# EricLBuehler/diffusion-rs

Measured on AMD Instinct MI355X. Metric: images/sec, FLUX.1-dev 1024x1024 50-step, higher is better.
Workload: dtype bf16; 1 GPU; FLUX.1-dev bf16 1024x1024 50-step, batch=1 per GPU, S=4096 img + T=512 txt tokens, step = one image (50x Flux::forward + Euler, unpack, VAE decode, u8); global_batch=1, parallelism=single GPU

## Files before the change

diffusion-rs_amd/_lib.py:

```python
import ctypes as C
import os

_HERE = os.path.dirname(os.path.abspath(__file__))
LIB_PATH = os.environ.get("FMI_LIB") or os.path.join(_HERE, "libflux_mi355x.so")
ALT_LIB_PATH = os.path.join(_HERE, "libflux_mi355x_alt.so")


class FmiError(RuntimeError):

    def __init__(self, msg, code=None):
        super().__init__(msg)
        self.code = code


ERR_INVALID, ERR_HIP, ERR_STATE, ERR_UNSUPPORTED, ERR_NOMEM = -1, -2, -3, -4, -5


class FluxConfig(C.Structure):
    _fields_ = [("in_channels", C.c_int), ("pooled_projection_dim", C.c_int), ("joint_attention_dim", C.c_int),
                ("num_attention_heads", C.c_int), ("num_layers", C.c_int), ("num_single_layers", C.c_int),
                ("guidance_embeds", C.c_int), ("axes_dim", C.c_int * 3), ("theta", C.c_int)]


ALL_TO_ALL_FN = C.CFUNCTYPE(C.c_int, C.c_void_p, C.c_void_p, C.c_void_p, C.c_size_t, C.c_void_p)
# ... 239 lines not shown
    lib.fmi_linear_int8_bf16.argtypes = [C.c_void_p, C.c_void_p, C.c_void_p, C.c_void_p, C.c_void_p, C.c_int, C.c_int, C.c_int, C.c_int, C.c_void_p]
    lib.fmi_sdpa_bf16.argtypes = [C.c_void_p, C.c_void_p, C.c_void_p, C.c_void_p, C.c_int, C.c_int, C.c_int, C.c_int, C.c_int, C.c_float, C.c_int,
                                  C.c_void_p]
    lib.fmi_sdpa_fp8qk.argtypes = lib.fmi_sdpa_bf16.argtypes
    lib.fmi_sdpa_workspace_bytes.argtypes = [C.c_int, C.c_int, C.c_int]
    lib.fmi_sdpa_workspace_bytes.restype = C.c_size_t
    lib.fmi_sdpa_bf16_ws.argtypes = [C.c_void_p] * 4 + [C.c_int] * 5 + [C.c_float, C.c_int, C.c_void_p, C.c_size_t, C.c_void_p]
    lib.fmi_sdpa_fp8qk_ws.argtypes = [C.c_void_p] * 4 + [C.c_int] * 5 + [C.c_float, C.c_int, C.c_int, C.c_void_p, C.c_size_t, C.c_void_p]
    lib.fmi_sdpa_fp8.argtypes = [C.c_void_p] * 4 + [C.c_int] * 5 + [C.c_float, C.c_int, C.c_float, C.c_int, C.c_void_p]
    lib.fmi_sdpa_fp8_ws.argtypes = [C.c_void_p] * 4 + [C.c_int] * 5 + [C.c_float, C.c_int, C.c_float, C.c_int, C.c_void_p, C.c_size_t, C.c_void_p]
    lib.fmi_linear_q8_workspace_bytes.argtypes = [C.c_int, C.c_int]
    lib.fmi_linear_q8_workspace_bytes.restype = C.c_size_t
    lib.fmi_linear_fp8_ws.argtypes = list(lib.fmi_linear_fp8.argtypes[:-1]) + [C.c_void_p, C.c_size_t, C.c_void_p]
    lib.fmi_linear_i8_ws.argtypes = lib.fmi_linear_fp8_ws.argtypes
    lib.fmi_layernorm_mod.argtypes = [C.c_void_p, C.c_void_p, C.c_void_p, C.c_void_p, C.c_int, C.c_int, C.c_float, C.c_void_p]
    lib.fmi_groupnorm_nhwc.argtypes = [C.c_void_p, C.c_void_p, C.c_void_p, C.c_void_p, C.c_int, C.c_int, C.c_int, C.c_int, C.c_float, C.c_int,
                                       C.c_void_p]
    lib.fmi_conv2d_nhwc.argtypes = [C.c_void_p, C.c_void_p, C.c_void_p, C.c_void_p, C.c_void_p, C.c_int, C.c_int, C.c_int, C.c_int, C.c_int,
                                    C.c_int, C.c_int, C.c_void_p]
    for name in ("f32", "f16", "bf16"):
        for q in ("int8", "fp4", "nf4"):
            getattr(lib, f"dequantize_blockwise_{name}_{q}").argtypes = [C.c_void_p, C.c_void_p, C.c_void_p, C.c_void_p, C.c_int, C.c_int, C.c_void_p]
            getattr(lib, f"dequantize_blockwise_{name}_{q}").restype = None
        getattr(lib, f"dequantize_8bit_kernel_{name}").argtypes = [C.c_void_p, C.c_void_p, C.c_void_p, C.c_int, C.c_int, C.c_int]
        getattr(lib, f"dequantize_8bit_kernel_{name}").restype = None
    lib.fmi_event_create.argtypes = [C.POINTER(C.c_void_p)]
    lib.fmi_event_record.argtypes = [C.c_void_p, C.c_void_p]
    lib.fmi_event_elapsed_ms.argtypes = [C.c_void_p, C.c_void_p, C.POINTER(C.c_float)]
    lib.fmi_event_destroy.argtypes = [C.c_void_p]
    lib.fmi_stream_synchronize.argtypes = [C.c_void_p]
# ... 22 lines not shown


EXPORTED = [
    "fmi_last_error", "fmi_abi_version", "fmi_init", "fmi_device_info", "fmi_build_id", "fmi_has_alt_kernels", "fmi_flux_default_config", "fmi_flux_create", "fmi_flux_destroy",
    "fmi_flux_set_tensor", "fmi_flux_set_linear_bnb4", "fmi_flux_set_linear_int8", "fmi_flux_set_linear_gguf", "fmi_gguf_block_info", "fmi_gguf_dequantize", "fmi_flux_get_tensor", "fmi_flux_lora_add", "fmi_flux_lora_set_weight", "fmi_flux_lora_remove", "fmi_flux_lora_count", "fmi_flux_lora_name", "fmi_flux_set_quant_dense_cache", "fmi_flux_set_sequence_parallel", "fmi_flux_set_split_k", "fmi_set_bnb4_onewave_min_rows", "fmi_flux_set_attention_rescale_threshold", "fmi_flux_set_attention_kernel", "fmi_flux_state_buffer_count", "fmi_flux_state_export", "fmi_flux_state_adopt", "fmi_flux_state_buffer", "fmi_flux_set_modulation_gemm", "fmi_flux_quantize_fp8", "fmi_flux_quantize_int8", "fmi_flux_calibrate_int8", "fmi_flux_set_fp8_attention", "fmi_flux_missing_count", "fmi_flux_missing_name", "fmi_flux_size_in_bytes",
    "fmi_flux_forward", "fmi_flux_denoise", "fmi_flux_denoise_inpaint", "fmi_flux_forward_context", "fmi_flux_denoise_context", "fmi_flux_denoise_cached", "fmi_flux_step_cache_bytes", "fmi_flux_denoise_cfg", "fmi_flux_create_cond", "fmi_flux_cond_channels", "fmi_flux_forward_control", "fmi_flux_denoise_control", "fmi_flux_denoise_with",
    "fmi_flux_create_controlnet", "fmi_flux_is_controlnet", "fmi_flux_forward_controlnet", "fmi_flux_denoise_controlnet", "fmi_flux_controlnet_eval", "fmi_flux_controlnet_sample", "fmi_add_scaled_rows_bf16",
    "fmi_flux_set_profiling", "fmi_flux_set_fused_qkv_relayout", "fmi_flux_phase_count", "fmi_flux_phase_name", "fmi_flux_phase_ms",
    "fmi_vae_default_config", "fmi_vae_create", "fmi_vae_destroy", "fmi_vae_set_tensor", "fmi_vae_missing_count", "fmi_vae_missing_name",
    "fmi_vae_scale_factor", "fmi_vae_shift_factor", "fmi_vae_decode", "fmi_vae_encode", "fmi_vae_mid_attention",
    "fmi_t5_default_config", "fmi_t5_create", "fmi_t5_destroy", "fmi_t5_set_tensor", "fmi_t5_set_linear_bnb4", "fmi_t5_set_linear_int8", "fmi_t5_missing_count", "fmi_t5_missing_name",
    "fmi_t5_size_in_bytes", "fmi_t5_forward", "fmi_clip_default_config", "fmi_clip_create", "fmi_clip_destroy", "fmi_clip_set_tensor",
    "fmi_clip_missing_count", "fmi_clip_missing_name", "fmi_clip_size_in_bytes", "fmi_clip_forward", "fmi_pack_latents", "fmi_unpack_latents", "fmi_postprocess_u8",
    "fmi_preprocess_u8", "fmi_latent_mask", "fmi_encode_latents", "fmi_scale_noise", "fmi_latent_ids", "fmi_cfg_euler_step", "fmi_cast_cols_bf16", "fmi_mask_image", "fmi_fill_condition",
    "fmi_randn", "fmi_philox_u32", "fmi_calculate_shift", "fmi_get_timesteps", "fmi_linear_bf16", "fmi_linear_bnb4_bf16", "fmi_linear_int8_bf16", "fmi_quantize_rows_fp8", "fmi_linear_fp8", "fmi_quantize_rows_i8", "fmi_linear_i8", "fmi_gemm_q8", "fmi_quantize_rows_i8_asym", "fmi_rowsum_i8", "fmi_quantize_rows_i8_scaled", "fmi_col_absmax", "fmi_gemm_i8_asym", "fmi_gemm_group", "fmi_splitk_resid_gate", "fmi_set_gemm_kernel", "fmi_linear_q8_workspace_bytes", "fmi_linear_fp8_ws", "fmi_linear_i8_ws", "fmi_sdpa_bf16", "fmi_sdpa_fp8qk", "fmi_sdpa_workspace_bytes", "fmi_sdpa_bf16_ws", "fmi_sdpa_fp8qk_ws", "fmi_sdpa_fp8", "fmi_sdpa_fp8_ws", "fmi_set_attention_kernel", "fmi_layernorm_mod",
    "fmi_release_scratch", "fmi_timestep_embedding", "fmi_rope_table", "fmi_rmsnorm_rope",
    "fmi_groupnorm_nhwc", "fmi_conv2d_nhwc",
    "fmi_comm_probe", "fmi_comm_unique_id", "fmi_comm_create", "fmi_comm_destroy", "fmi_comm_rank", "fmi_comm_world_size", "fmi_comm_stats", "fmi_comm_all_to_all",
    "fmi_comm_broadcast", "fmi_comm_gather",
    "dequantize_blockwise_f32_int8", "dequantize_blockwise_f32_fp4", "dequantize_blockwise_f32_nf4", "dequantize_blockwise_f16_int8",
    "dequantize_blockwise_f16_fp4", "dequantize_blockwise_f16_nf4", "dequantize_blockwise_bf16_int8", "dequantize_blockwise_bf16_fp4",
    "dequantize_blockwise_bf16_nf4", "dequantize_8bit_kernel_f32", "dequantize_8bit_kernel_f16", "dequantize_8bit_kernel_bf16",
    "fmi_malloc", "fmi_free", "fmi_memcpy", "fmi_memset", "fmi_stream_synchronize", "fmi_event_create", "fmi_event_record",
    "fmi_event_elapsed_ms", "fmi_event_destroy",
]
```

diffusion-rs_amd/csrc/capi.hip:

```cpp
#include <algorithm>
#include <cmath>
#include <cstring>
#include <map>
#include <mutex>
#include <set>
#include <thread>
#include <tuple>
#include <utility>
#include <vector>

#include "common.h"

namespace fmi {
static thread_local std::string g_err;
void set_error(const std::string& msg) { g_err = msg; }
int fail(fmi_status st, const std::string& msg) {
  g_err = msg;
  return (int)st;
}
}
using namespace fmi;

extern "C" const char* fmi_last_error(void) { return g_err.c_str(); }
extern "C" int fmi_abi_version(void) { return FMI_ABI_VERSION; }
// ... 467 lines not shown
  return fmi_sdpa_fp8_ws(q, k, v, o, B, H, Lq, Lk, d, scale, score_exp2, v_scale, out_token_major, ws.p, bytes, stream);
}

extern "C" int fmi_set_attention_kernel(int kind) {
  if (kind < 0 || kind > 5) return fail(FMI_ERR_INVALID, "set_attention_kernel: kind must be 0 .. 5");
  if (!alt_kernels_built() && kind != 5 && kind != 1)
    return fail(FMI_ERR_UNSUPPORTED, "set_attention_kernel: this build carries kernels 5 and 1; 0, 2, 3, 4 live in the test build (libflux_mi355x_alt.so: make alt)");
  set_attention_kind(kind);
  return FMI_OK;
}

extern "C" int fmi_layernorm_mod(const float* x, const float* scale, const float* shift, void* out_bf16, int rows, int D, float eps, void* stream) {
  if (!x || !out_bf16) return fail(FMI_ERR_INVALID, "layernorm_mod: null pointer");
  return launch_layernorm_mod(x, scale, shift, 0, 0, (bf16_t*)out_bf16, rows, D, eps, (hipStream_t)stream);
}

extern "C" int fmi_timestep_embedding(const float* t, int B, int dim, float* out, void* stream) {
  if (!t || !out) return fail(FMI_ERR_INVALID, "timestep_embedding: null pointer");
  if (B <= 0 || dim <= 0 || dim % 2) return fail(FMI_ERR_INVALID, "timestep_embedding: B > 0 and an even dim > 0 required");
  return launch_timestep_embedding(t, B, dim, out, (hipStream_t)stream);
}
extern "C" int fmi_rope_table(const float* txt_ids, const float* img_ids, int B, int T, int S, const int* axes_dim, int theta, float* pe, void* stream) {
  if (!axes_dim || !pe || (T > 0 && !txt_ids) || (S > 0 && !img_ids)) return fail(FMI_ERR_INVALID, "rope_table: null pointer");
  if (B <= 0 || T < 0 || S < 0 || T + S == 0) return fail(FMI_ERR_INVALID, "rope_table: empty problem");
  for (int a = 0; a < 3; ++a)
    if (axes_dim[a] <= 0 || axes_dim[a] % 2) return fail(FMI_ERR_INVALID, "rope_table: every axes_dim must be positive and even");
  if (theta <= 0) return fail(FMI_ERR_INVALID, "rope_table: theta must be positive");
  return launch_rope_table(txt_ids, img_ids, B, T, S, axes_dim, theta, pe, (hipStream_t)stream);
}
extern "C" int fmi_rmsnorm_rope(const void* q, const void* k, int ld, const void* q_weight, const void* k_weight, const float* pe, void* q_out, void* k_out,
// ... 18 lines not shown
```

diffusion-rs_amd/csrc/common.h:

```cpp
#pragma once
#ifndef FMI_ALT_KERNELS
#define FMI_ALT_KERNELS 0
#endif
#include <type_traits>
#include <hip/hip_runtime.h>
#include <stdint.h>

#include <set>
#include <string>
#include <vector>

#include "../../include/flux_mi355x.h"

namespace fmi {

void set_error(const std::string& msg);
int fail(fmi_status st, const std::string& msg);
#define FMI_HIP_TRY(expr)                                                                       \
  do {                                                                                          \
    hipError_t _e = (expr);                                                                     \
    if (_e != hipSuccess)                                                                       \
      return ::fmi::fail(FMI_ERR_HIP, std::string(#expr) + ": " + hipGetErrorString(_e) + " @" + \
                                          __FILE__ + ":" + std::to_string(__LINE__));           \
  } while (0)
// ... 306 lines not shown
                        const bf16_t* wk, const float* pe, int64_t pe_bstride, bf16_t* qo, bf16_t* ko,
                        int B, int H, int rows, int row_off, int Ltot, hipStream_t stream);
int launch_qk_norm_rope_f32(const bf16_t* q, const bf16_t* k, int ld, int64_t in_bstride, const bf16_t* wq, const bf16_t* wk, const float* pe,
                            int64_t pe_bstride, float* qo, float* ko, int B, int H, int rows, int row_off, int Ltot, hipStream_t stream);
int launch_rope_table(const float* txt_ids, const float* img_ids, int B, int T, int S, const int* axes,
                      int theta, float* pe, hipStream_t stream, const float* ctx_ids = nullptr, int R = 0);
int launch_layernorm_mod2(const float* x, const float* scale, const float* shift, int mod_bstride, int rows_per_batch, bf16_t* out, int rows,
                          const float* x2, const float* scale2, const float* shift2, int rows_per_batch2, bf16_t* out2, int rows2, int D, float eps,
                          hipStream_t stream);
int launch_layernorm_mod_fp8_2(const float* x, const float* scale, const float* shift, int mod_bstride, int rows_per_batch, uint8_t* out,
                               float* out_scale, int rows, const float* x2, const float* scale2, const float* shift2, int rows_per_batch2, uint8_t* out2,
                               float* out_scale2, int rows2, int D, float eps, hipStream_t stream, int kind = 1, const float* smooth = nullptr,
                               const float* smooth2 = nullptr);
int launch_layernorm_mod(const float* x, const float* scale, const float* shift, int mod_bstride,
                         int rows_per_batch, bf16_t* out, int rows, int D, float eps, hipStream_t stream);
int launch_quantize_rows_fp8(const bf16_t* x, int ld, int rows, int K, uint8_t* out, float* scale, hipStream_t stream, int kind = 1, const float* vec = nullptr);
int launch_quantize_rows_i8_asym(const bf16_t* x, int ld, int rows, int K, int d0, uint8_t* out, float* scale, float* offset, hipStream_t stream, const float* vec = nullptr);
int launch_rowsum_i8(const int8_t* wq, const float* w_scale, int N, int K, int d0, float* w_sum, hipStream_t stream);
int launch_layernorm_mod_fp8(const float* x, const float* scale, const float* shift, int mod_bstride, int rows_per_batch,
                             uint8_t* out, float* out_scale, int rows, int D, float eps, hipStream_t stream, int kind = 1, const float* smooth = nullptr);
int launch_col_absmax(const bf16_t* x, int ld, int rows, int K, float* amax, hipStream_t stream);
void smooth_factors_host(const float* act_amax, const float* w_amax, int K, float* s_out, float* inv_out);
int launch_gemv(const float* x, const bf16_t* W, const bf16_t* bias, float* y, int M, int N, int K,
                int silu_in, int accumulate, hipStream_t stream);
int launch_dequant_int8_scb_bf16(const int8_t* w, const float* scb, bf16_t* out, int col, int64_t n, hipStream_t stream);
constexpr int LORA_TILE_ROWS = 64, LORA_RANK_CHUNK = 16;
int launch_lora_pack(const float* A, const float* B, int rows, int K, int r, double coef, float* Acat, double* Bt, int rows_pad, int off, hipStream_t stream);
int launch_lora_merge(const bf16_t* w0, bf16_t* w, int rows, int K, const float* A, const double* Bt, int rows_pad, int Rpad, hipStream_t stream);
int launch_timestep_embedding(const float* t, int B, int dim, float* out, hipStream_t stream);
int launch_cast_to_bf16(const void* src, fmi_dtype dt, bf16_t* dst, int64_t n, hipStream_t stream);
// ... 22 lines not shown
```

diffusion-rs_amd/csrc/fp8.hip:

```cpp
#include <algorithm>
#include <cmath>
#include <vector>

#include "common.h"

namespace fmi {

namespace {

constexpr float kE4M3Max = 448.0f;
constexpr float kI8Max = 127.0f;

__device__ __forceinline__ float block_max_256(float v, float* red) {
  v = wave_max(v);
  if ((threadIdx.x & 63) == 0) red[threadIdx.x >> 6] = v;
  __syncthreads();
  return fmaxf(fmaxf(red[0], red[1]), fmaxf(red[2], red[3]));
}

__device__ __forceinline__ uint32_t pack_e4m3x4(float a, float b, float c, float d) {
  int v = 0;
  v = __builtin_amdgcn_cvt_pk_fp8_f32(a, b, v, false);
  v = __builtin_amdgcn_cvt_pk_fp8_f32(c, d, v, true);
  return (uint32_t)v;
// ... 128 lines not shown
  const int4* r = reinterpret_cast<const int4*>(wq + (int64_t)n * K);
  int t = 0;
  for (int i = (d0 >> 4) + lane; i < (K >> 4); i += 64) {
    const int4 x = r[i];
    const int w[4] = {x.x, x.y, x.z, x.w};
#pragma unroll
    for (int e = 0; e < 4; ++e) t += (int)(int8_t)(w[e] & 0xff) + (int)(int8_t)((w[e] >> 8) & 0xff) + (int)(int8_t)((w[e] >> 16) & 0xff) + (w[e] >> 24);
  }
#pragma unroll
  for (int o = 32; o > 0; o >>= 1) t += __shfl_xor(t, o);
  if (lane == 0) w_sum[n] = w_scale[n] * (float)t;
}

constexpr int LN_MAXV = 4;

template <bool I8>
__global__ __launch_bounds__(256) void layernorm_mod_fp8_kernel(const float* __restrict x1, const float* __restrict scale1,
                                                                const float* __restrict shift1, int mod_bstride, int rows_per_batch1,
                                                                uint8_t* __restrict out1, float* __restrict out_scale1, int D, float eps, int rows1,
                                                                const float* __restrict x2, const float* __restrict scale2,
                                                                const float* __restrict shift2, int rows_per_batch2, uint8_t* __restrict out2,
                                                                float* __restrict out_scale2, const float* __restrict smooth1,
                                                                const float* __restrict smooth2) {
  __shared__ float red[2][4];
  __shared__ float redm[4];
  const bool second = (int)blockIdx.x >= rows1;
  const int row = second ? blockIdx.x - rows1 : blockIdx.x;
  const float* x = second ? x2 : x1;
  const float* scale = second ? scale2 : scale1;
  const float* shift = second ? shift2 : shift1;
// ... 53 lines not shown
      v[c] = make_float4(a, b, cc, d);
      am = fmaxf(fmaxf(am, fmaxf(fabsf(a), fabsf(b))), fmaxf(fabsf(cc), fabsf(d)));
    }
  }
  am = fmaxf(block_max_256(am, redm), 1e-30f);
  constexpr float QMAX = I8 ? kI8Max : kE4M3Max;
  const float inv = QMAX / am;
  if (threadIdx.x == 0) out_scale[row] = am / QMAX;
  uint32_t* o = reinterpret_cast<uint32_t*>(out + (int64_t)row * D);
#pragma unroll
  for (int c = 0; c < LN_MAXV; ++c) {
    const int i = threadIdx.x + c * 256;
    if (i < nv) o[i] = pack_q8x4<I8>(v[c].x * inv, v[c].y * inv, v[c].z * inv, v[c].w * inv);
  }
}


__global__ __launch_bounds__(256) void col_absmax_kernel(const bf16_t* __restrict x, int ld, int rows, int chunks, float* __restrict amax) {
  const int i = blockIdx.x * 256 + threadIdx.x;
  if (i >= chunks) return;
  float m[8] = {0.f, 0.f, 0.f, 0.f, 0.f, 0.f, 0.f, 0.f};
  for (int r = blockIdx.y; r < rows; r += gridDim.y) {
    const uint4 raw = *reinterpret_cast<const uint4*>(x + (int64_t)r * ld + 8 * i);
    float f[8];
    widen8<false>(raw, nullptr, 0, f);
#pragma unroll
    for (int e = 0; e < 8; ++e) m[e] = fmaxf(m[e], fabsf(f[e]));
  }
#pragma unroll
  for (int e = 0; e < 8; ++e)
// ... 26 lines not shown
}
int launch_rowsum_i8(const int8_t* wq, const float* w_scale, int N, int K, int d0, float* w_sum, hipStream_t stream) {
  if (N <= 0) return FMI_OK;
  if (K % 16 || d0 % 16 || d0 < 0 || d0 > K) return fail(FMI_ERR_INVALID, "rowsum_i8: K and d0 must be multiples of 16");
  hipLaunchKernelGGL(rowsum_i8_kernel, dim3((N + 3) / 4), dim3(256), 0, stream, wq, w_scale, N, K, d0, w_sum);
  FMI_LAUNCH_CHECK();
  return FMI_OK;
}

int launch_layernorm_mod_fp8_2(const float* x, const float* scale, const float* shift, int mod_bstride, int rows_per_batch, uint8_t* out,
                               float* out_scale, int rows, const float* x2, const float* scale2, const float* shift2, int rows_per_batch2, uint8_t* out2,
                               float* out_scale2, int rows2, int D, float eps, hipStream_t stream, int kind, const float* smooth, const float* smooth2) {
  if (rows + rows2 <= 0) return FMI_OK;
  if (kind != 1 && kind != 2) return fail(FMI_ERR_INVALID, "layernorm_mod_fp8: kind must be 1 (e4m3) or 2 (int8)");
  if (D % 4 || D > 256 * 4 * LN_MAXV) return fail(FMI_ERR_INVALID, "layernorm_mod_fp8: D must be a multiple of 4 and <= 4096");
  if (kind == 2)
    hipLaunchKernelGGL(layernorm_mod_fp8_kernel<true>, dim3(rows + rows2), dim3(256), 0, stream, x, scale, shift, mod_bstride, rows_per_batch, out, out_scale,
                       D, eps, rows, x2, scale2, shift2, rows_per_batch2, out2, out_scale2, smooth, smooth2);
  else
    hipLaunchKernelGGL(layernorm_mod_fp8_kernel<false>, dim3(rows + rows2), dim3(256), 0, stream, x, scale, shift, mod_bstride, rows_per_batch, out, out_scale,
                       D, eps, rows, x2, scale2, shift2, rows_per_batch2, out2, out_scale2, smooth, smooth2);
  FMI_LAUNCH_CHECK();
  return FMI_OK;
}
int launch_layernorm_mod_fp8(const float* x, const float* scale, const float* shift, int mod_bstride, int rows_per_batch, uint8_t* out,
                             float* out_scale, int rows, int D, float eps, hipStream_t stream, int kind, const float* smooth) {
  return launch_layernorm_mod_fp8_2(x, scale, shift, mod_bstride, rows_per_batch, out, out_scale, rows, nullptr, nullptr, nullptr, 0, nullptr, nullptr, 0,
                                    D, eps, stream, kind, smooth, nullptr);
}

int launch_col_absmax(const bf16_t* x, int ld, int rows, int K, float* amax, hipStream_t stream) {
  if (rows <= 0 || K <= 0) return FMI_OK;
  if (K % 8 || ld % 8) return fail(FMI_ERR_INVALID, "col_absmax: K and ld must be multiples of 8");
  const int chunks = K / 8, rblocks = std::min((rows + 63) / 64, 512);
  hipLaunchKernelGGL(col_absmax_kernel, dim3((chunks + 255) / 256, rblocks), dim3(256), 0, stream, x, ld, rows, chunks, amax);
  FMI_LAUNCH_CHECK();
// ... 21 lines not shown
```

diffusion-rs_amd/csrc/norm_rope.hip:

```cpp
#include "common.h"

namespace fmi {

template <bool REG>
__global__ __launch_bounds__(256) void layernorm_mod_kernel(const float* __restrict x1, const float* __restrict scale1,
                                                            const float* __restrict shift1, int mod_bstride, int rows_per_batch1,
                                                            bf16_t* __restrict out1, int D, float eps, int rows1, const float* __restrict x2,
                                                            const float* __restrict scale2, const float* __restrict shift2, int rows_per_batch2,
                                                            bf16_t* __restrict out2) {
  __shared__ float red[2][4];
  const bool second = (int)blockIdx.x >= rows1;
  const int row = second ? blockIdx.x - rows1 : blockIdx.x;
  const float* x = second ? x2 : x1;
  const float* scale = second ? scale2 : scale1;
  const float* shift = second ? shift2 : shift1;
  const int rows_per_batch = second ? rows_per_batch2 : rows_per_batch1;
  bf16_t* out = second ? out2 : out1;
  const float4* xr = reinterpret_cast<const float4*>(x + (int64_t)row * D);
  const int nv = D >> 2;
  constexpr int MAXV = 4;
  float4 keep[MAXV], ksc[MAXV], ksh[MAXV];
  float s = 0.f, s2 = 0.f;
  const int batch = rows_per_batch > 0 ? row / rows_per_batch : 0;
  const float4* sc = scale ? reinterpret_cast<const float4*>(scale + (int64_t)batch * mod_bstride) : nullptr;
// ... 50 lines not shown
    }
    o[i] = make_uint2(pack_bf16x2(a, b), pack_bf16x2(c, d));
  };
  if constexpr (REG) {
#pragma unroll
    for (int c = 0; c < MAXV; ++c) {
      const int i = threadIdx.x + c * 256;
      if (i < nv) emit(i, keep[c], ksc[c], ksh[c]);
    }
  } else {
    const float4 z = make_float4(0.f, 0.f, 0.f, 0.f);
    for (int i = threadIdx.x; i < nv; i += 256) emit(i, xr[i], sc ? sc[i] : z, sh ? sh[i] : z);
  }
}

int launch_layernorm_mod2(const float* x, const float* scale, const float* shift, int mod_bstride, int rows_per_batch, bf16_t* out, int rows,
                          const float* x2, const float* scale2, const float* shift2, int rows_per_batch2, bf16_t* out2, int rows2, int D, float eps,
                          hipStream_t stream) {
  if (rows + rows2 <= 0) return FMI_OK;
  if (D % 4) return fail(FMI_ERR_INVALID, "layernorm_mod: D must be a multiple of 4");
  if (D <= 4096)
    hipLaunchKernelGGL(layernorm_mod_kernel<true>, dim3(rows + rows2), dim3(256), 0, stream, x, scale, shift, mod_bstride, rows_per_batch, out, D, eps, rows,
                       x2, scale2, shift2, rows_per_batch2, out2);
  else
    hipLaunchKernelGGL(layernorm_mod_kernel<false>, dim3(rows + rows2), dim3(256), 0, stream, x, scale, shift, mod_bstride, rows_per_batch, out, D, eps, rows,
                       x2, scale2, shift2, rows_per_batch2, out2);
  FMI_LAUNCH_CHECK();
  return FMI_OK;
}
int launch_layernorm_mod(const float* x, const float* scale, const float* shift, int mod_bstride, int rows_per_batch, bf16_t* out,
                         int rows, int D, float eps, hipStream_t stream) {
  return launch_layernorm_mod2(x, scale, shift, mod_bstride, rows_per_batch, out, rows, nullptr, nullptr, nullptr, 0, nullptr, 0, D, eps, stream);
}

template <bool F32OUT>
__global__ __launch_bounds__(256) void qk_norm_rope_kernel(const bf16_t* __restrict q, const bf16_t* __restrict k, int ld,
                                                           int64_t in_bstride, const bf16_t* __restrict wq,
                                                           const bf16_t* __restrict wk, const float* __restrict pe,
                                                           int64_t pe_bstride, void* __restrict qo, void* __restrict ko, int B,
                                                           int H, int rows, int row_off, int Ltot) {
  const int64_t gid = (int64_t)blockIdx.x * 16 + (threadIdx.x >> 4);
// ... 109 lines not shown
```

include/flux_mi355x.h:

```cpp
#ifndef FLUX_MI355X_H
#define FLUX_MI355X_H

#include <stddef.h>
#include <stdint.h>

#ifdef __cplusplus
extern "C" {
#endif
#pragma GCC visibility push(default)

#define FMI_ABI_VERSION 6

typedef enum fmi_status {
  FMI_OK = 0,
  FMI_ERR_INVALID = -1,
  FMI_ERR_HIP = -2,
  FMI_ERR_STATE = -3,
  FMI_ERR_UNSUPPORTED = -4,
  FMI_ERR_NOMEM = -5
} fmi_status;

typedef enum fmi_dtype {
  FMI_F32 = 0,
  FMI_F16 = 1,
// ... 345 lines not shown
int fmi_release_scratch(size_t* freed_bytes);
int fmi_sdpa_bf16_ws(const void* q, const void* k, const void* v, void* o, int B, int H, int Lq, int Lk, int d, float scale,
                     int out_token_major, void* workspace, size_t workspace_bytes, void* stream);
int fmi_set_attention_kernel(int kind);
int fmi_sdpa_fp8qk(const void* q, const void* k, const void* v, void* o, int B, int H, int Lq,
                  int Lk, int d, float scale, int out_token_major, void* stream);
#define FMI_SDPA_NO_EXP2 (1 << 30)
int fmi_sdpa_fp8qk_ws(const void* q, const void* k, const void* v, void* o, int B, int H, int Lq, int Lk, int d, float scale,
                      int score_exp2, int out_token_major, void* workspace, size_t workspace_bytes, void* stream);
int fmi_sdpa_fp8(const void* q, const void* k, const void* v, void* o, int B, int H, int Lq, int Lk, int d, float scale, int score_exp2,
                 float v_scale, int out_token_major, void* stream);
int fmi_sdpa_fp8_ws(const void* q, const void* k, const void* v, void* o, int B, int H, int Lq, int Lk, int d, float scale, int score_exp2,
                    float v_scale, int out_token_major, void* workspace, size_t workspace_bytes, void* stream);
int fmi_layernorm_mod(const float* x, const float* scale, const float* shift, void* out_bf16,
                      int rows, int D, float eps, void* stream);
int fmi_timestep_embedding(const float* t, int B, int dim, float* out, void* stream);
int fmi_rope_table(const float* txt_ids, const float* img_ids, int B, int T, int S, const int* axes_dim , int theta, float* pe, void* stream);
int fmi_rmsnorm_rope(const void* q, const void* k, int ld, const void* q_weight, const void* k_weight, const float* pe, void* q_out, void* k_out,
                     int B, int H, int L, int d, fmi_dtype out_dtype, void* stream);
int fmi_groupnorm_nhwc(const void* x_bf16, const float* weight, const float* bias, void* out_bf16,
                       int B, int HW, int C, int groups, float eps, int fuse_silu, void* stream);
int fmi_conv2d_nhwc(const void* x_bf16, const void* w_bf16, const void* bias_bf16,
                    const void* residual_bf16, void* out_bf16, int B, int in_h, int in_w, int Cin,
                    int Cout, int ksize, int upsample2x, void* stream);

void dequantize_blockwise_f32_int8(const float* code, const uint8_t* A, const float* absmax, float* out, int blocksize, int n, void* stream);
void dequantize_blockwise_f32_fp4(const float* code, const uint8_t* A, const float* absmax, float* out, int blocksize, int n, void* stream);
void dequantize_blockwise_f32_nf4(const float* code, const uint8_t* A, const float* absmax, float* out, int blocksize, int n, void* stream);
void dequantize_blockwise_f16_int8(const float* code, const uint8_t* A, const float* absmax, void* out, int blocksize, int n, void* stream);
void dequantize_blockwise_f16_fp4(const float* code, const uint8_t* A, const float* absmax, void* out, int blocksize, int n, void* stream);
// ... 24 lines not shown
```

Baseline: 0.3262 images/s.

## Process multiple rows per block in modulated layernorm with prefetch of next row

Replaces the one-row-per-block modulated layernorm (bf16 and fp8/int8 quantizing variants) with a persistent grid sized from the CU count, where each block walks a contiguous range of rows. It prefetches the next row into registers while reducing the current one and caches the per-batch scale/shift vectors across rows. The aim is to cut per-block launch and scheduling overhead and to overlap memory loads with the reductions. The old kernels are moved into the alt build, and new C API entry points and tuning knobs are added. The cost is more register pressure and possible load imbalance.

```diff
diff --git a/diffusion-rs_amd/_lib.py b/diffusion-rs_amd/_lib.py
--- a/diffusion-rs_amd/_lib.py
+++ b/diffusion-rs_amd/_lib.py
@@ -277,6 +277,13 @@
     lib.fmi_linear_fp8_ws.argtypes = list(lib.fmi_linear_fp8.argtypes[:-1]) + [C.c_void_p, C.c_size_t, C.c_void_p]
     lib.fmi_linear_i8_ws.argtypes = lib.fmi_linear_fp8_ws.argtypes
     lib.fmi_layernorm_mod.argtypes = [C.c_void_p, C.c_void_p, C.c_void_p, C.c_void_p, C.c_int, C.c_int, C.c_float, C.c_void_p]
+    ln_set = [C.c_void_p, C.c_void_p, C.c_void_p]
+    lib.fmi_layernorm_mod2.argtypes = ln_set + [C.c_int, C.c_int, C.c_void_p, C.c_int] + ln_set + [C.c_int, C.c_void_p, C.c_int, C.c_int, C.c_float, C.c_void_p]
+    lib.fmi_layernorm_mod2_q8.argtypes = (ln_set + [C.c_int, C.c_int, C.c_void_p, C.c_void_p, C.c_int] + ln_set + [C.c_int, C.c_void_p, C.c_void_p, C.c_int, C.c_int, C.c_float, C.c_int,
+                                          C.c_void_p, C.c_void_p, C.c_void_p])
+    lib.fmi_set_layernorm_kernel.argtypes = [C.c_int, C.c_float]
+    lib.fmi_layernorm_grid.argtypes = [C.c_int, C.c_int, C.c_int, C.POINTER(C.c_int), C.POINTER(C.c_int)]
+    lib.fmi_layernorm_block_rows.argtypes = [C.c_int, C.c_int, C.c_void_p, C.c_void_p]
     lib.fmi_groupnorm_nhwc.argtypes = [C.c_void_p, C.c_void_p, C.c_void_p, C.c_void_p, C.c_int, C.c_int, C.c_int, C.c_int, C.c_float, C.c_int,
                                        C.c_void_p]
     lib.fmi_conv2d_nhwc.argtypes = [C.c_void_p, C.c_void_p, C.c_void_p, C.c_void_p, C.c_void_p, C.c_int, C.c_int, C.c_int, C.c_int, C.c_int,
@@ -329,6 +336,7 @@
     "fmi_clip_missing_count", "fmi_clip_missing_name", "fmi_clip_size_in_bytes", "fmi_clip_forward", "fmi_pack_latents", "fmi_unpack_latents", "fmi_postprocess_u8",
     "fmi_preprocess_u8", "fmi_latent_mask", "fmi_encode_latents", "fmi_scale_noise", "fmi_latent_ids", "fmi_cfg_euler_step", "fmi_cast_cols_bf16", "fmi_mask_image", "fmi_fill_condition",
     "fmi_randn", "fmi_philox_u32", "fmi_calculate_shift", "fmi_get_timesteps", "fmi_linear_bf16", "fmi_linear_bnb4_bf16", "fmi_linear_int8_bf16", "fmi_quantize_rows_fp8", "fmi_linear_fp8", "fmi_quantize_rows_i8", "fmi_linear_i8", "fmi_gemm_q8", "fmi_quantize_rows_i8_asym", "fmi_rowsum_i8", "fmi_quantize_rows_i8_scaled", "fmi_col_absmax", "fmi_gemm_i8_asym", "fmi_gemm_group", "fmi_splitk_resid_gate", "fmi_set_gemm_kernel", "fmi_linear_q8_workspace_bytes", "fmi_linear_fp8_ws", "fmi_linear_i8_ws", "fmi_sdpa_bf16", "fmi_sdpa_fp8qk", "fmi_sdpa_workspace_bytes", "fmi_sdpa_bf16_ws", "fmi_sdpa_fp8qk_ws", "fmi_sdpa_fp8", "fmi_sdpa_fp8_ws", "fmi_set_attention_kernel", "fmi_layernorm_mod",
+    "fmi_layernorm_mod2", "fmi_layernorm_mod2_q8", "fmi_set_layernorm_kernel", "fmi_layernorm_grid", "fmi_layernorm_block_rows",
     "fmi_release_scratch", "fmi_timestep_embedding", "fmi_rope_table", "fmi_rmsnorm_rope",
     "fmi_groupnorm_nhwc", "fmi_conv2d_nhwc",
     "fmi_comm_probe", "fmi_comm_unique_id", "fmi_comm_create", "fmi_comm_destroy", "fmi_comm_rank", "fmi_comm_world_size", "fmi_comm_stats", "fmi_comm_all_to_all",
diff --git a/diffusion-rs_amd/csrc/capi.hip b/diffusion-rs_amd/csrc/capi.hip
--- a/diffusion-rs_amd/csrc/capi.hip
+++ b/diffusion-rs_amd/csrc/capi.hip
@@ -505,6 +505,44 @@
   if (!x || !out_bf16) return fail(FMI_ERR_INVALID, "layernorm_mod: null pointer");
   return launch_layernorm_mod(x, scale, shift, 0, 0, (bf16_t*)out_bf16, rows, D, eps, (hipStream_t)stream);
 }
+extern "C" int fmi_layernorm_mod2(const float* x, const float* scale, const float* shift, int mod_bstride, int rows_per_batch, void* out_bf16, int rows,
+                                  const float* x2, const float* scale2, const float* shift2, int rows_per_batch2, void* out2_bf16, int rows2, int D, float eps,
+                                  void* stream) {
+  if (rows < 0 || rows2 < 0 || rows_per_batch < 0 || rows_per_batch2 < 0) return fail(FMI_ERR_INVALID, "layernorm_mod2: negative row count");
+  if ((rows > 0 && (!x || !out_bf16)) || (rows2 > 0 && (!x2 || !out2_bf16))) return fail(FMI_ERR_INVALID, "layernorm_mod2: null pointer");
+  if (mod_bstride % 4 || ((reinterpret_cast<uintptr_t>(scale) | reinterpret_cast<uintptr_t>(shift) | reinterpret_cast<uintptr_t>(scale2) | reinterpret_cast<uintptr_t>(shift2)) & 15))
+    return fail(FMI_ERR_INVALID, "layernorm_mod2: scale / shift must be 16-byte aligned and mod_bstride a multiple of 4 elements (read as float4)");
+  return launch_layernorm_mod2(x, scale, shift, mod_bstride, rows_per_batch, (bf16_t*)out_bf16, rows, x2, scale2, shift2, rows_per_batch2, (bf16_t*)out2_bf16, rows2,
+                               D, eps, (hipStream_t)stream);
+}
+extern "C" int fmi_layernorm_mod2_q8(const float* x, const float* scale, const float* shift, int mod_bstride, int rows_per_batch, uint8_t* out_q8, float* out_scale,
+                                     int rows, const float* x2, const float* scale2, const float* shift2, int rows_per_batch2, uint8_t* out2_q8, float* out_scale2,
+                                     int rows2, int D, float eps, int kind, const float* smooth, const float* smooth2, void* stream) {
+  if (rows < 0 || rows2 < 0 || rows_per_batch < 0 || rows_per_batch2 < 0) return fail(FMI_ERR_INVALID, "layernorm_mod2_q8: negative row count");
+  if ((rows > 0 && (!x || !out_q8 || !out_scale)) || (rows2 > 0 && (!x2 || !out2_q8 || !out_scale2))) return fail(FMI_ERR_INVALID, "layernorm_mod2_q8: null pointer");
+  if (mod_bstride % 4 || ((reinterpret_cast<uintptr_t>(scale) | reinterpret_cast<uintptr_t>(shift) | reinterpret_cast<uintptr_t>(scale2) | reinterpret_cast<uintptr_t>(shift2) |
+                            reinterpret_cast<uintptr_t>(smooth) | reinterpret_cast<uintptr_t>(smooth2)) & 15))
+    return fail(FMI_ERR_INVALID, "layernorm_mod2_q8: scale / shift / smooth must be 16-byte aligned and mod_bstride a multiple of 4 elements (read as float4)");
+  return launch_layernorm_mod_fp8_2(x, scale, shift, mod_bstride, rows_per_batch, out_q8, out_scale, rows, x2, scale2, shift2, rows_per_batch2, out2_q8, out_scale2, rows2,
+                                    D, eps, (hipStream_t)stream, kind, smooth, smooth2);
+}
+extern "C" int fmi_set_layernorm_kernel(int rowblock, float rows_per_block) {
+  if (!(rows_per_block >= 0.f)) return fail(FMI_ERR_INVALID, "set_layernorm_kernel: rows_per_block must be >= 0 (0: the grid function chooses)");
+  set_layernorm_rowblock(rowblock != 0, (double)rows_per_block);
+  return FMI_OK;
+}
+extern "C" int fmi_layernorm_grid(int rows, int D, int cus, int* blocks, int* rows_per_block) {
+  if (rows < 0 || D <= 0 || D > 4096 || !blocks || !rows_per_block) return fail(FMI_ERR_INVALID, "layernorm_grid: rows >= 0, 0 < D <= 4096 and both outputs required");
+  if (cus <= 0 && (cus = device_cu_count()) <= 0) return fail(FMI_ERR_HIP, "layernorm_grid: cannot read the device's CU count");
+  const LnGrid g = ln_row_grid(rows, cus, ln_resident_blocks_for(D), layernorm_rows_pin());
+  *blocks = g.blocks, *rows_per_block = g.rows_per_block;
+  return FMI_OK;
+}
+extern "C" int fmi_layernorm_block_rows(int rows, int blocks, int* first, int* end) {
+  if (rows < 0 || blocks <= 0 || !first || !end) return fail(FMI_ERR_INVALID, "layernorm_block_rows: rows >= 0, blocks > 0 and both outputs required");
+  ln_block_rows(rows, blocks, first, end);
+  return FMI_OK;
+}
 
 extern "C" int fmi_timestep_embedding(const float* t, int B, int dim, float* out, void* stream) {
   if (!t || !out) return fail(FMI_ERR_INVALID, "timestep_embedding: null pointer");
diff --git a/diffusion-rs_amd/csrc/common.h b/diffusion-rs_amd/csrc/common.h
--- a/diffusion-rs_amd/csrc/common.h
+++ b/diffusion-rs_amd/csrc/common.h
@@ -344,6 +344,28 @@
                                const float* smooth2 = nullptr);
 int launch_layernorm_mod(const float* x, const float* scale, const float* shift, int mod_bstride,
                          int rows_per_batch, bf16_t* out, int rows, int D, float eps, hipStream_t stream);
+enum LnKernel {
+  LK_ROW_BLOCKS,
+  LK_ROW_REG,
+  LK_ROW_TWO_PASS,
+};
+struct LnChoice {
+  LnKernel kernel;
+  fmi_status err;
+  const char* msg;
+};
+LnChoice select_layernorm_kernel(int D, bool rowblock, bool alt);
+__host__ __device__ inline int ln_block_first(int rows, int blocks, int b) { return (int)((int64_t)b * rows / blocks); }
+struct LnGrid {
+  int blocks, rows_per_block;
+};
+LnGrid ln_row_grid(int rows, int cus, int resident, double pin_rows);
+int ln_resident_blocks_for(int D);
+bool layernorm_rowblock();
+void ln_block_rows(int rows, int blocks, int* first, int* end);
+void set_layernorm_rowblock(bool on, double pin_rows);
+double layernorm_rows_pin();
+int device_cu_count();
 int launch_quantize_rows_fp8(const bf16_t* x, int ld, int rows, int K, uint8_t* out, float* scale, hipStream_t stream, int kind = 1, const float* vec = nullptr);
 int launch_quantize_rows_i8_asym(const bf16_t* x, int ld, int rows, int K, int d0, uint8_t* out, float* scale, float* offset, hipStream_t stream, const float* vec = nullptr);
 int launch_rowsum_i8(const int8_t* wq, const float* w_scale, int N, int K, int d0, float* w_sum, hipStream_t stream);
diff --git a/diffusion-rs_amd/csrc/fp8.hip b/diffusion-rs_amd/csrc/fp8.hip
--- a/diffusion-rs_amd/csrc/fp8.hip
+++ b/diffusion-rs_amd/csrc/fp8.hip
@@ -166,6 +166,7 @@
 
 constexpr int LN_MAXV = 4;
 
+#if FMI_ALT_KERNELS
 template <bool I8>
 __global__ __launch_bounds__(256) void layernorm_mod_fp8_kernel(const float* __restrict x1, const float* __restrict scale1,
                                                                 const float* __restrict shift1, int mod_bstride, int rows_per_batch1,
@@ -249,6 +250,125 @@
     if (i < nv) o[i] = pack_q8x4<I8>(v[c].x * inv, v[c].y * inv, v[c].z * inv, v[c].w * inv);
   }
 }
+#endif
+
+constexpr int lnq_resident_blocks(int nc, bool smooth) { return (nc < 4 ? 6 : 5) - (smooth ? 1 : 0); }
+template <bool I8, int NC, bool EXACT, bool SMOOTH>
+__global__ __launch_bounds__(256, lnq_resident_blocks(NC, SMOOTH)) void layernorm_mod_fp8_rows_kernel(
+    const float* __restrict x1, const float* __restrict scale1, const float* __restrict shift1, int mod_bstride, int rows_per_batch1, uint8_t* __restrict out1,
+    float* __restrict out_scale1, int D, float eps, int rows1, const float* __restrict x2, const float* __restrict scale2, const float* __restrict shift2,
+    int rows_per_batch2, uint8_t* __restrict out2, float* __restrict out_scale2, const float* __restrict smooth1, const float* __restrict smooth2,
+    int rows_total) {
+  __shared__ float red[2][2][4];
+  __shared__ float redm[2][4];
+  const int g0 = ln_block_first(rows_total, gridDim.x, blockIdx.x), g1 = ln_block_first(rows_total, gridDim.x, blockIdx.x + 1);
+  if (g0 >= g1) return;
+  const int nv = D >> 2;
+  float4 cur[NC], nxt[NC], ksc[NC], ksh[NC], ksm[SMOOTH ? NC : 1];
+  const int w = threadIdx.x >> 6;
+  auto owns = [&](int i) { return EXACT || i < nv; };
+  auto load_row = [&](int g, float4(&keep)[NC]) {
+    const bool second = g >= rows1;
+    const float4* xr = reinterpret_cast<const float4*>((second ? x2 : x1) + (int64_t)(second ? g - rows1 : g) * D);
+#pragma unroll
+    for (int c = 0; c < NC; ++c) {
+      const int i = threadIdx.x + c * 256;
+      if (owns(i)) keep[c] = xr[i];
+    }
+  };
+  int have_set = -1, have_batch = -1;
+  auto do_row = [&](int g, float4(&v)[NC], auto more) {
+    constexpr bool MORE = decltype(more)::value;
+    const bool second = g >= rows1;
+    const int row = second ? g - rows1 : g;
+    const float* scale = second ? scale2 : scale1;
+    const float* shift = second ? shift2 : shift1;
+    const int rows_per_batch = second ? rows_per_batch2 : rows_per_batch1;
+    uint8_t* out = second ? out2 : out1;
+    float* out_scale = second ? out_scale2 : out_scale1;
+    const float4* sm = SMOOTH ? reinterpret_cast<const float4*>(second ? smooth2 : smooth1) : nullptr;
+    const int batch = rows_per_batch > 0 ? row / rows_per_batch : 0;
+    const float4* sc = scale ? reinterpret_cast<const float4*>(scale + (int64_t)batch * mod_bstride) : nullptr;
+    const float4* sh = shift ? reinterpret_cast<const float4*>(shift + (int64_t)batch * mod_bstride) : nullptr;
+    if ((int)second != have_set || batch != have_batch) {
+      have_set = (int)second, have_batch = batch;
+#pragma unroll
+      for (int c = 0; c < NC; ++c) {
+        const int i = threadIdx.x + c * 256;
+        if (owns(i)) {
+          if (sc) ksc[c] = sc[i];
+          if (sh) ksh[c] = sh[i];
+          if constexpr (SMOOTH)
+            if (sm) ksm[c] = sm[i];
+        }
+      }
+    }
+    if constexpr (MORE) load_row(g + 1, nxt);
+    float s = 0.f, s2 = 0.f;
+#pragma unroll
+    for (int c = 0; c < NC; ++c) {
+      const int i = threadIdx.x + c * 256;
+      if (owns(i)) {
+        s += (v[c].x + v[c].y) + (v[c].z + v[c].w);
+        s2 += (v[c].x * v[c].x + v[c].y * v[c].y) + (v[c].z * v[c].z + v[c].w * v[c].w);
+      }
+    }
+    s = wave_sum(s);
+    s2 = wave_sum(s2);
+    const int par = (g - g0) & 1;
+    if ((threadIdx.x & 63) == 0) {
+      red[par][0][w] = s;
+      red[par][1][w] = s2;
+    }
+    __syncthreads();
+    s = (red[par][0][0] + red[par][0][1]) + (red[par][0][2] + red[par][0][3]);
+    s2 = (red[par][1][0] + red[par][1][1]) + (red[par][1][2] + red[par][1][3]);
+    const float mean = s / (float)D;
+    const float var = s2 / (float)D - mean * mean;
+    const float inv_std = 1.0f / sqrtf(var + eps);
+    float am = 0.f;
+#pragma unroll
+    for (int c = 0; c < NC; ++c) {
+      const int i = threadIdx.x + c * 256;
+      if (owns(i)) {
+        float a = (v[c].x - mean) * inv_std, b = (v[c].y - mean) * inv_std, cc = (v[c].z - mean) * inv_std, d = (v[c].w - mean) * inv_std;
+        if (sc) {
+          const float4 k = ksc[c];
+          a *= (k.x + 1.0f), b *= (k.y + 1.0f), cc *= (k.z + 1.0f), d *= (k.w + 1.0f);
+        }
+        if (sh) {
+          const float4 k = ksh[c];
+          a += k.x, b += k.y, cc += k.z, d += k.w;
+        }
+        if constexpr (SMOOTH) {
+          if (sm) {
+            const float4 k = ksm[c];
+            a *= k.x, b *= k.y, cc *= k.z, d *= k.w;
+          }
+        }
+        v[c] = make_float4(a, b, cc, d);
+        am = fmaxf(fmaxf(am, fmaxf(fabsf(a), fabsf(b))), fmaxf(fabsf(cc), fabsf(d)));
+      }
+    }
+    am = fmaxf(block_max_256(am, redm[par]), 1e-30f);
+    constexpr float QMAX = I8 ? kI8Max : kE4M3Max;
+    const float inv = QMAX / am;
+    if (threadIdx.x == 0) out_scale[row] = am / QMAX;
+    uint32_t* o = reinterpret_cast<uint32_t*>(out + (int64_t)row * D);
+#pragma unroll
+    for (int c = 0; c < NC; ++c) {
+      const int i = threadIdx.x + c * 256;
+      if (owns(i)) o[i] = pack_q8x4<I8>(v[c].x * inv, v[c].y * inv, v[c].z * inv, v[c].w * inv);
+    }
+  };
+  load_row(g0, cur);
+  for (int g = g0; g + 1 < g1; ++g) {
+    do_row(g, cur, std::true_type{});
+#pragma unroll
+    for (int c = 0; c < NC; ++c) cur[c] = nxt[c];
+  }
+  do_row(g1 - 1, cur, std::false_type{});
+}
 
 
 __global__ __launch_bounds__(256) void col_absmax_kernel(const bf16_t* __restrict x, int ld, int rows, int chunks, float* __restrict amax) {
@@ -305,12 +425,40 @@
   if (rows + rows2 <= 0) return FMI_OK;
   if (kind != 1 && kind != 2) return fail(FMI_ERR_INVALID, "layernorm_mod_fp8: kind must be 1 (e4m3) or 2 (int8)");
   if (D % 4 || D > 256 * 4 * LN_MAXV) return fail(FMI_ERR_INVALID, "layernorm_mod_fp8: D must be a multiple of 4 and <= 4096");
-  if (kind == 2)
-    hipLaunchKernelGGL(layernorm_mod_fp8_kernel<true>, dim3(rows + rows2), dim3(256), 0, stream, x, scale, shift, mod_bstride, rows_per_batch, out, out_scale,
-                       D, eps, rows, x2, scale2, shift2, rows_per_batch2, out2, out_scale2, smooth, smooth2);
-  else
-    hipLaunchKernelGGL(layernorm_mod_fp8_kernel<false>, dim3(rows + rows2), dim3(256), 0, stream, x, scale, shift, mod_bstride, rows_per_batch, out, out_scale,
-                       D, eps, rows, x2, scale2, shift2, rows_per_batch2, out2, out_scale2, smooth, smooth2);
+  const LnChoice c = select_layernorm_kernel(D, layernorm_rowblock(), FMI_ALT_KERNELS != 0);
+  if (c.err != FMI_OK) return fail(c.err, c.msg);
+  if (c.kernel == LK_ROW_BLOCKS) {
+    const int cus = device_cu_count();
+    if (cus <= 0) return fail(FMI_ERR_HIP, "layernorm_mod_fp8: cannot read the device's CU count");
+    const bool sm = smooth || smooth2;
+    const int nc = D == 3072 ? 3 : 4;
+    const LnGrid g = ln_row_grid(rows + rows2, cus, lnq_resident_blocks(nc, sm), layernorm_rows_pin());
+    auto launch = [&](auto kernel) {
+      hipLaunchKernelGGL(kernel, dim3(g.blocks), dim3(256), 0, stream, x, scale, shift, mod_bstride, rows_per_batch, out, out_scale, D, eps, rows, x2, scale2,
+                         shift2, rows_per_batch2, out2, out_scale2, smooth, smooth2, rows + rows2);
+    };
+    auto by_shape = [&](auto i8, auto smoothed) {
+      constexpr bool I8 = decltype(i8)::value, SM = decltype(smoothed)::value;
+      if (D == 3072) launch(layernorm_mod_fp8_rows_kernel<I8, 3, true, SM>);
+      else if (D == 4096) launch(layernorm_mod_fp8_rows_kernel<I8, 4, true, SM>);
+      else launch(layernorm_mod_fp8_rows_kernel<I8, 4, false, SM>);
+    };
+    if (kind == 2 && sm) by_shape(std::true_type{}, std::true_type{});
+    else if (kind == 2) by_shape(std::true_type{}, std::false_type{});
+    else if (sm) by_shape(std::false_type{}, std::true_type{});
+    else by_shape(std::false_type{}, std::false_type{});
+  } else {
+#if FMI_ALT_KERNELS
+    if (kind == 2)
+      hipLaunchKernelGGL(layernorm_mod_fp8_kernel<true>, dim3(rows + rows2), dim3(256), 0, stream, x, scale, shift, mod_bstride, rows_per_batch, out, out_scale,
+                         D, eps, rows, x2, scale2, shift2, rows_per_batch2, out2, out_scale2, smooth, smooth2);
+    else
+      hipLaunchKernelGGL(layernorm_mod_fp8_kernel<false>, dim3(rows + rows2), dim3(256), 0, stream, x, scale, shift, mod_bstride, rows_per_batch, out, out_scale,
+                         D, eps, rows, x2, scale2, shift2, rows_per_batch2, out2, out_scale2, smooth, smooth2);
+#else
+    return fail(FMI_ERR_UNSUPPORTED, "layernorm_mod_fp8: the selected kernel is not part of this build");
+#endif
+  }
   FMI_LAUNCH_CHECK();
   return FMI_OK;
 }
diff --git a/diffusion-rs_amd/csrc/norm_rope.hip b/diffusion-rs_amd/csrc/norm_rope.hip
--- a/diffusion-rs_amd/csrc/norm_rope.hip
+++ b/diffusion-rs_amd/csrc/norm_rope.hip
@@ -1,4 +1,9 @@
 #include "common.h"
+
+#include <algorithm>
+#include <atomic>
+#include <cmath>
+#include <cstdlib>
 
 namespace fmi {
 
@@ -88,17 +93,211 @@
   }
 }
 
+
+constexpr int ln_resident_blocks(int nc) { return nc < 4 ? 6 : 5; }
+int ln_resident_blocks_for(int D) { return ln_resident_blocks(D % 1024 ? 4 : D / 1024); }
+
+constexpr double LN_ROW_LATENCY = 2.2;
+LnGrid ln_row_grid(int rows, int cus, int resident, double pin_rows) {
+  LnGrid g{0, 0};
+  if (rows <= 0) return g;
+  if (cus <= 0) cus = 1;
+  auto with_blocks = [&](int64_t blocks) {
+    g.blocks = (int)std::max<int64_t>(1, std::min<int64_t>(blocks, rows));
+    g.rows_per_block = (rows + g.blocks - 1) / g.blocks;
+    return g;
+  };
+  if (pin_rows > 0) return with_blocks((int64_t)std::ceil(rows / pin_rows));
+  if (rows <= cus) return with_blocks(rows);
+  int best = 0;
+  double best_cost = 1e300;
+  auto consider = [&](int blocks) {
+    const int k = (blocks + cus - 1) / cus;
+    const int r = (rows + blocks - 1) / blocks;
+    const double cu_rows = std::min<double>((double)k * r, (double)rows / cus + (rows % blocks ? r : 0));
+    const double cost = std::max(1.5 * cu_rows, LN_ROW_LATENCY * (r + 1));
+    if (cost < best_cost + 1e-9) best_cost = std::min(cost, best_cost), best = blocks;
+  };
+  for (int k = 1; k <= resident && (int64_t)k * cus <= rows; ++k) consider(k * cus);
+  if ((int64_t)rows <= (int64_t)resident * cus) consider(rows);
+  return with_blocks(best);
+}
+void ln_block_rows(int rows, int blocks, int* first, int* end) {
+  for (int b = 0; b < blocks; ++b) first[b] = ln_block_first(rows, blocks, b), end[b] = ln_block_first(rows, blocks, b + 1);
+}
+
+template <int NC, bool EXACT>
+__global__ __launch_bounds__(256, ln_resident_blocks(NC)) void layernorm_mod_rows_kernel(const float* __restrict x1, const float* __restrict scale1,
+                                                                                     const float* __restrict shift1, int mod_bstride, int rows_per_batch1,
+                                                                                     bf16_t* __restrict out1, int D, float eps, int rows1,
+                                                                                     const float* __restrict x2, const float* __restrict scale2,
+                                                                                     const float* __restrict shift2, int rows_per_batch2,
+                                                                                     bf16_t* __restrict out2, int rows_total) {
+  __shared__ float red[2][2][4];
+  const int g0 = ln_block_first(rows_total, gridDim.x, blockIdx.x), g1 = ln_block_first(rows_total, gridDim.x, blockIdx.x + 1);
+  if (g0 >= g1) return;
+  const int nv = D >> 2;
+  constexpr int MAXV = NC;
+  float4 cur[MAXV], nxt[MAXV], ksc[MAXV], ksh[MAXV];
+  const int w = threadIdx.x >> 6;
+  auto owns = [&](int i) { return EXACT || i < nv; };
+  auto row_ptr = [&](int g) {
+    const bool second = g >= rows1;
+    return reinterpret_cast<const float4*>((second ? x2 : x1) + (int64_t)(second ? g - rows1 : g) * D);
+  };
+  auto load_row = [&](int g, float4(&keep)[MAXV]) {
+    const float4* xr = row_ptr(g);
+#pragma unroll
+    for (int c = 0; c < MAXV; ++c) {
+      const int i = threadIdx.x + c * 256;
+      if (owns(i)) keep[c] = xr[i];
+    }
+  };
+  int have_set = -1, have_batch = -1;
+  auto do_row = [&](int g, float4(&keep)[MAXV], auto more) {
+    constexpr bool MORE = decltype(more)::value;
+    const bool second = g >= rows1;
+    const int row = second ? g - rows1 : g;
+    const float* scale = second ? scale2 : scale1;
+    const float* shift = second ? shift2 : shift1;
+    const int rows_per_batch = second ? rows_per_batch2 : rows_per_batch1;
+    bf16_t* out = second ? out2 : out1;
+    const int batch = rows_per_batch > 0 ? row / rows_per_batch : 0;
+    const float4* sc = scale ? reinterpret_cast<const float4*>(scale + (int64_t)batch * mod_bstride) : nullptr;
+    const float4* sh = shift ? reinterpret_cast<const float4*>(shift + (int64_t)batch * mod_bstride) : nullptr;
+    if ((int)second != have_set || batch != have_batch) {
+      have_set = (int)second, have_batch = batch;
+#pragma unroll
+      for (int c = 0; c < MAXV; ++c) {
+        const int i = threadIdx.x + c * 256;
+        if (owns(i)) {
+          if (sc) ksc[c] = sc[i];
+          if (sh) ksh[c] = sh[i];
+        }
+      }
+    }
+    if constexpr (MORE) load_row(g + 1, nxt);
+    float s = 0.f, s2 = 0.f;
+#pragma unroll
+    for (int c = 0; c < MAXV; ++c) {
+      const int i = threadIdx.x + c * 256;
+      if (owns(i)) {
+        const float4 v = keep[c];
+        s += (v.x + v.y) + (v.z + v.w);
+        s2 += (v.x * v.x + v.y * v.y) + (v.z * v.z + v.w * v.w);
+      }
+    }
+    s = wave_sum(s);
+    s2 = wave_sum(s2);
+    float(&rd)[2][4] = red[(g - g0) & 1];
+    if ((threadIdx.x & 63) == 0) {
+      rd[0][w] = s;
+      rd[1][w] = s2;
+    }
+    __syncthreads();
+    s = (rd[0][0] + rd[0][1]) + (rd[0][2] + rd[0][3]);
+    s2 = (rd[1][0] + rd[1][1]) + (rd[1][2] + rd[1][3]);
+    const float mean = s / (float)D;
+    const float var = s2 / (float)D - mean * mean;
+    const float inv_std = 1.0f / sqrtf(var + eps);
+    uint2* o = reinterpret_cast<uint2*>(out + (int64_t)row * D);
+#pragma unroll
+    for (int c = 0; c < MAXV; ++c) {
+      const int i = threadIdx.x + c * 256;
+      if (owns(i)) {
+        const float4 v = keep[c];
+        float a = (v.x - mean) * inv_std, b = (v.y - mean) * inv_std, cc = (v.z - mean) * inv_std, d = (v.w - mean) * inv_std;
+        if (sc) {
+          const float4 k = ksc[c];
+          a *= (k.x + 1.0f);
+          b *= (k.y + 1.0f);
+          cc *= (k.z + 1.0f);
+          d *= (k.w + 1.0f);
+        }
+        if (sh) {
+          const float4 k = ksh[c];
+          a += k.x;
+          b += k.y;
+          cc += k.z;
+          d += k.w;
+        }
+        o[i] = make_uint2(pack_bf16x2(a, b), pack_bf16x2(cc, d));
+      }
+    }
+  };
+  load_row(g0, cur);
+  for (int g = g0; g + 1 < g1; ++g) {
+    do_row(g, cur, std::true_type{});
+#pragma unroll
+    for (int c = 0; c < MAXV; ++c) cur[c] = nxt[c];
+  }
+  do_row(g1 - 1, cur, std::false_type{});
+}
+
+LnChoice select_layernorm_kernel(int D, bool rowblock, bool alt) {
+  if (D > 4096) return {LK_ROW_TWO_PASS, FMI_OK, nullptr};
+  if (rowblock) return {LK_ROW_BLOCKS, FMI_OK, nullptr};
+  if (!alt)
+    return {LK_ROW_BLOCKS, FMI_ERR_UNSUPPORTED, "layernorm_mod: the one-row-per-block kernel (FMI_LN_ROWBLOCK=0) lives in the test build (libflux_mi355x_alt.so: make alt)"};
+  return {LK_ROW_REG, FMI_OK, nullptr};
+}
+static std::atomic<bool> g_ln_rowblock{[] {
+  const char* e = getenv("FMI_LN_ROWBLOCK");
+  return !(e && atoi(e) == 0);
+}()};
+static std::atomic<double> g_ln_rows_pin{[] {
+  const char* e = getenv("FMI_LN_ROWS");
+  return e ? atof(e) : 0.0;
+}()};
+void set_layernorm_rowblock(bool on, double pin_rows) { g_ln_rowblock = on, g_ln_rows_pin = pin_rows > 0 ? pin_rows : 0.0; }
+double layernorm_rows_pin() { return g_ln_rows_pin; }
+bool layernorm_rowblock() { return g_ln_rowblock; }
+int device_cu_count() {
+  static const int cus = [] {
+    int dev = 0, n = 0;
+    if (hipGetDevice(&dev) != hipSuccess || hipDeviceGetAttribute(&n, hipDeviceAttributeMultiprocessorCount, dev) != hipSuccess) return 0;
+    return n;
+  }();
+  return cus;
+}
+
 int launch_layernorm_mod2(const float* x, const float* scale, const float* shift, int mod_bstride, int rows_per_batch, bf16_t* out, int rows,
                           const float* x2, const float* scale2, const float* shift2, int rows_per_batch2, bf16_t* out2, int rows2, int D, float eps,
                           hipStream_t stream) {
   if (rows + rows2 <= 0) return FMI_OK;
   if (D % 4) return fail(FMI_ERR_INVALID, "layernorm_mod: D must be a multiple of 4");
-  if (D <= 4096)
-    hipLaunchKernelGGL(layernorm_mod_kernel<true>, dim3(rows + rows2), dim3(256), 0, stream, x, scale, shift, mod_bstride, rows_per_batch, out, D, eps, rows,
-                       x2, scale2, shift2, rows_per_batch2, out2);
-  else
-    hipLaunchKernelGGL(layernorm_mod_kernel<false>, dim3(rows + rows2), dim3(256), 0, stream, x, scale, shift, mod_bstride, rows_per_batch, out, D, eps, rows,
-                       x2, scale2, shift2, rows_per_batch2, out2);
+  const LnChoice c = select_layernorm_kernel(D, g_ln_rowblock, FMI_ALT_KERNELS != 0);
+  if (c.err != FMI_OK) return fail(c.err, c.msg);
+  switch (c.kernel) {
+    case LK_ROW_BLOCKS: {
+      const int cus = device_cu_count();
+      if (cus <= 0) return fail(FMI_ERR_HIP, "layernorm_mod: cannot read the device's CU count");
+      const LnGrid g = ln_row_grid(rows + rows2, cus, ln_resident_blocks_for(D), layernorm_rows_pin());
+      auto launch = [&](auto kernel) {
+        hipLaunchKernelGGL(kernel, dim3(g.blocks), dim3(256), 0, stream, x, scale, shift, mod_bstride, rows_per_batch, out, D, eps, rows, x2, scale2, shift2,
+                           rows_per_batch2, out2, rows + rows2);
+      };
+      switch (D % 1024 ? 0 : D / 1024) {
+        case 1: launch(layernorm_mod_rows_kernel<1, true>); break;
+        case 2: launch(layernorm_mod_rows_kernel<2, true>); break;
+        case 3: launch(layernorm_mod_rows_kernel<3, true>); break;
+        case 4: launch(layernorm_mod_rows_kernel<4, true>); break;
+        default: launch(layernorm_mod_rows_kernel<4, false>); break;
+      }
+      break;
+    }
+    case LK_ROW_TWO_PASS:
+      hipLaunchKernelGGL(layernorm_mod_kernel<false>, dim3(rows + rows2), dim3(256), 0, stream, x, scale, shift, mod_bstride, rows_per_batch, out, D, eps,
+                         rows, x2, scale2, shift2, rows_per_batch2, out2);
+      break;
+#if FMI_ALT_KERNELS
+    case LK_ROW_REG:
+      hipLaunchKernelGGL(layernorm_mod_kernel<true>, dim3(rows + rows2), dim3(256), 0, stream, x, scale, shift, mod_bstride, rows_per_batch, out, D, eps,
+                         rows, x2, scale2, shift2, rows_per_batch2, out2);
+      break;
+#endif
+    default: return fail(FMI_ERR_UNSUPPORTED, "layernorm_mod: the selected kernel is not part of this build");
+  }
   FMI_LAUNCH_CHECK();
   return FMI_OK;
 }
diff --git a/include/flux_mi355x.h b/include/flux_mi355x.h
--- a/include/flux_mi355x.h
+++ b/include/flux_mi355x.h
@@ -383,6 +383,15 @@
                     float v_scale, int out_token_major, void* workspace, size_t workspace_bytes, void* stream);
 int fmi_layernorm_mod(const float* x, const float* scale, const float* shift, void* out_bf16,
                       int rows, int D, float eps, void* stream);
+int fmi_layernorm_mod2(const float* x, const float* scale, const float* shift, int mod_bstride, int rows_per_batch, void* out_bf16, int rows,
+                       const float* x2, const float* scale2, const float* shift2, int rows_per_batch2, void* out2_bf16, int rows2, int D, float eps,
+                       void* stream);
+int fmi_layernorm_mod2_q8(const float* x, const float* scale, const float* shift, int mod_bstride, int rows_per_batch, uint8_t* out_q8, float* out_scale,
+                          int rows, const float* x2, const float* scale2, const float* shift2, int rows_per_batch2, uint8_t* out2_q8, float* out_scale2,
+                          int rows2, int D, float eps, int kind, const float* smooth, const float* smooth2, void* stream);
+int fmi_set_layernorm_kernel(int rowblock, float rows_per_block);
+int fmi_layernorm_grid(int rows, int D, int cus, int* blocks, int* rows_per_block);
+int fmi_layernorm_block_rows(int rows, int blocks, int* first, int* end);
 int fmi_timestep_embedding(const float* t, int B, int dim, float* out, void* stream);
 int fmi_rope_table(const float* txt_ids, const float* img_ids, int B, int T, int S, const int* axes_dim , int theta, float* pe, void* stream);
 int fmi_rmsnorm_rope(const void* q, const void* k, int ld, const void* q_weight, const void* k_weight, const float* pe, void* q_out, void* k_out,
```

Result: no change. 0.3272 images/s (median of 6 runs) (+0.3%).
